# bennevans/mjrl

Hardware: AMD Instinct MI355X
Metric: NPG train_step timesteps/sec, Humanoid 1M-step batch @ 1/2/4/8 MI355X (higher is better)
Workload: dtype f32 (split-f16 MFMA, f32 accumulate); 1 GPU; humanoid_npg_1M; obs_dim=376, act_dim=17, algo=npg, horizon=1000, cg_iters=10, parallelism=dp1, comm=LocalComm

## Files before the change

### mjrl_amd/csrc/common.h

```cpp
#pragma once

#include <hip/hip_runtime.h>
#include <stdint.h>

#include "../../include/mjrl_amd.h"

#ifdef MJRL_KX_PROF
constexpr int KX_NPROF = 24;
__device__ unsigned long long g_kx_prof[KX_NPROF];
#define KX_STAMP(i)                                                     \
    do {                                                                \
        const unsigned long long now_ = __builtin_amdgcn_s_memtime();   \
        kx_acc_[i] += now_ - kx_last_;                                  \
        kx_last_ = now_;                                                \
    } while (0)
#define KX_PRE(i) kx_pre_[i] = __builtin_amdgcn_s_memtime()
#else
#define KX_PRE(i) \
    do {          \
    } while (0)
#define KX_STAMP(i) \
    do {            \
    } while (0)
#endif

namespace mjrl {

typedef float floatx4 __attribute__((ext_vector_type(4)));

constexpr int WAVE = 64;
constexpr int NTHREADS = 256;

__device__ __forceinline__ floatx4 zero4() { return floatx4{0.f, 0.f, 0.f, 0.f}; }

__device__ __forceinline__ floatx4 mfma4(float a, float b, floatx4 c) {
    return __builtin_amdgcn_mfma_f32_16x16x4f32(a, b, c, 0, 0, 0);
}

__device__ __forceinline__ floatx4 mfma_k16(const float4& a, const float4& b, floatx4 c) {
    c = mfma4(a.x, b.x, c);
    c = mfma4(a.y, b.y, c);
    c = mfma4(a.z, b.z, c);
    c = mfma4(a.w, b.w, c);
    return c;
}

typedef _Float16 half8 __attribute__((ext_vector_type(8)));
typedef short short4v __attribute__((ext_vector_type(4)));

__device__ __forceinline__ floatx4 mfma_h(const half8& a, const half8& b, floatx4 c) {
    return __builtin_amdgcn_mfma_f32_16x16x32_f16(a, b, c, 0, 0, 0);
}

__device__ __forceinline__ floatx4 mfma_x3(const half8& ah, const half8& al, const half8& bh, const half8& bl,
                                           floatx4 c) {
    c = mfma_h(ah, bh, c);
    c = mfma_h(ah, bl, c);
    return mfma_h(al, bh, c);
}

constexpr int SPLIT_HR = 15;

__device__ __forceinline__ float pow2_scale(float M, float& inv) {
    if (!(M > 0.f) || !(M < 3.0e38f)) {
        inv = 1.f;
        return 1.f;
    }
    int E;
    frexpf(M, &E);
    E = E < -111 ? -111 : E;
    inv = ldexpf(1.f, E - SPLIT_HR);
    return ldexpf(1.f, SPLIT_HR - E);
}

__device__ __forceinline__ float col_scale(float cmax) {
    if (!(cmax > 0.f) || !(cmax < 3.0e38f)) return 1.f;
    int E;
    frexpf(cmax, &E);
    E = E < -100 ? -100 : (E > 100 ? 100 : E);
    return ldexpf(1.f, E);
}

constexpr float AHR = 16384.f;
constexpr float AHR_INV = 1.f / 16384.f;

typedef float float8v __attribute__((ext_vector_type(8)));
typedef short short8v __attribute__((ext_vector_type(8)));

typedef unsigned uint4v __attribute__((ext_vector_type(4)));

__device__ __forceinline__ uint4v mix_lo8(const uint4v& h, const float8v& y) {
    uint4v l;
    asm("v_fma_mixlo_f16 %0, %4, -1.0, %8 op_sel_hi:[1,0,0]\n\t"
        "v_fma_mixhi_f16 %0, %4, -1.0, %9 op_sel:[1,0,0] op_sel_hi:[1,0,0]\n\t"
        "v_fma_mixlo_f16 %1, %5, -1.0, %10 op_sel_hi:[1,0,0]\n\t"
        "v_fma_mixhi_f16 %1, %5, -1.0, %11 op_sel:[1,0,0] op_sel_hi:[1,0,0]\n\t"
        "v_fma_mixlo_f16 %2, %6, -1.0, %12 op_sel_hi:[1,0,0]\n\t"
        "v_fma_mixhi_f16 %2, %6, -1.0, %13 op_sel:[1,0,0] op_sel_hi:[1,0,0]\n\t"
        "v_fma_mixlo_f16 %3, %7, -1.0, %14 op_sel_hi:[1,0,0]\n\t"
        "v_fma_mixhi_f16 %3, %7, -1.0, %15 op_sel:[1,0,0] op_sel_hi:[1,0,0]\n\t"
        "s_nop 1"
        : "=&v"(l[0]), "=&v"(l[1]), "=&v"(l[2]), "=&v"(l[3])
        : "v"(h[0]), "v"(h[1]), "v"(h[2]), "v"(h[3]), "v"(y[0]), "v"(y[1]), "v"(y[2]), "v"(y[3]), "v"(y[4]),
          "v"(y[5]), "v"(y[6]), "v"(y[7]));
    return l;
}

__device__ __forceinline__ unsigned mix_lo2(unsigned hi2, float y0, float y1) {
    unsigned t;
    asm("v_fma_mixlo_f16 %0, %1, -1.0, %2 op_sel_hi:[1,0,0]\n\t"
        "v_fma_mixhi_f16 %0, %1, -1.0, %3 op_sel:[1,0,0] op_sel_hi:[1,0,0]"
        : "=&v"(t) : "v"(hi2), "v"(y0), "v"(y1));
    return t;
}

__device__ __forceinline__ void split8(const float8v& v, float s, half8& hi, half8& lo) {
    const float8v y = v * s;
    hi = __builtin_convertvector(y, half8);
    lo = __builtin_bit_cast(half8, mix_lo8(__builtin_bit_cast(uint4v, hi), y));
}

__device__ __forceinline__ float mix_add_lo(unsigned h2, unsigned l2) {
    float r;
    asm("v_fma_mix_f32 %0, %1, 1.0, %2 op_sel_hi:[1,0,1]" : "=v"(r) : "v"(h2), "v"(l2));
    return r;
}
__device__ __forceinline__ float mix_add_hi(unsigned h2, unsigned l2) {
    float r;
    asm("v_fma_mix_f32 %0, %1, 1.0, %2 op_sel:[1,0,1] op_sel_hi:[1,0,1]" : "=v"(r) : "v"(h2), "v"(l2));
    return r;
}
__device__ __forceinline__ float8v hilo8(const half8& hh, const half8& ll) {
    const uint4v h = __builtin_bit_cast(uint4v, hh), l = __builtin_bit_cast(uint4v, ll);
    float8v r;
#pragma unroll
    for (int p = 0; p < 4; ++p) {
        r[2 * p] = mix_add_lo(h[p], l[p]);
        r[2 * p + 1] = mix_add_hi(h[p], l[p]);
    }
    return r;
}

__device__ __forceinline__ float8v load8(const float* p) {
    const float4 a = *reinterpret_cast<const float4*>(p);
    const float4 b = *reinterpret_cast<const float4*>(p + 4);
    return float8v{a.x, a.y, a.z, a.w, b.x, b.y, b.z, b.w};
}

__device__ __forceinline__ float absmax8(const float8v& v) {
    float m = 0.f;
#pragma unroll
    for (int e = 0; e < 8; ++e) m = fmaxf(m, fabsf(v[e]));
    return m;
}

__device__ __forceinline__ float max_over_groups(float v) {
    const auto a = __builtin_amdgcn_permlane16_swap(__float_as_uint(v), __float_as_uint(v), false, false);
    v = fmaxf(__uint_as_float(a[0]), __uint_as_float(a[1]));
    const auto b = __builtin_amdgcn_permlane32_swap(__float_as_uint(v), __float_as_uint(v), false, false);
    return fmaxf(__uint_as_float(b[0]), __uint_as_float(b[1]));
}

__device__ __forceinline__ float sum_over_groups(float v) {
    const auto a = __builtin_amdgcn_permlane16_swap(__float_as_uint(v), __float_as_uint(v), false, false);
    v = __uint_as_float(a[0]) + __uint_as_float(a[1]);
    const auto b = __builtin_amdgcn_permlane32_swap(__float_as_uint(v), __float_as_uint(v), false, false);
    return __uint_as_float(b[0]) + __uint_as_float(b[1]);
}

__device__ __forceinline__ short4v ds_read_tr16(const void* p) {
    typedef __attribute__((address_space(3))) short4v lds_short4;
    return __builtin_amdgcn_ds_read_tr16_b64_v4i16((lds_short4*)(p));
}

template <int RB, int CB, int NW = 4>
struct Split {
    static constexpr int WPC = CB >= NW ? 1 : NW / CB;
    static constexpr int NCW = CB >= NW ? CB / NW : 1;
    static constexpr int NRW = CB >= NW ? RB : (RB + WPC - 1) / WPC;
    static constexpr int CBS = CB >= NW ? NW : 1;
    static constexpr int RBS = CB >= NW ? 1 : WPC;
    __device__ static int cb0(int w) { return CB >= NW ? w : w % CB; }
    __device__ static int rb0(int w) { return CB >= NW ? 0 : w / CB; }
};

template <int NRW, int NCW>
__device__ __forceinline__ void gemm_tile(floatx4 (&acc)[NRW][NCW], const float* As, int lda, int a_col0,
                                          int rb0, int rbs, int rb_lim, const float* __restrict__ W, int ldw,
                                          int cb0, int cbs, int kb, int ke, int lane) {
    const int r = lane & 15, q = lane >> 4;
#ifndef MJRL_GEMM_UNROLL
#define MJRL_GEMM_UNROLL 8
#endif
#pragma unroll MJRL_GEMM_UNROLL
    for (int k = kb; k < ke; k += 16) {
        float4 b[NCW];
#pragma unroll
        for (int j = 0; j < NCW; ++j)
            b[j] = *reinterpret_cast<const float4*>(W + (size_t)((cb0 + j * cbs) * 16 + r) * ldw + k + 4 * q);
#pragma unroll
        for (int i = 0; i < NRW; ++i) {
            const int rb = rb0 + i * rbs;
            if (rb >= rb_lim) continue;
            const float4 a = *reinterpret_cast<const float4*>(As + (rb * 16 + r) * lda + (k - a_col0) + 4 * q);
#pragma unroll
            for (int j = 0; j < NCW; ++j) acc[i][j] = mfma_k16(a, b[j], acc[i][j]);
        }
    }
}

template <int NRW, int NCW>
__device__ __forceinline__ void zero_acc(floatx4 (&acc)[NRW][NCW]) {
#pragma unroll
// ... 174 lines not shown
```

### mjrl_amd/csrc/kx.h

```cpp
#pragma once


namespace {

constexpr int AIMG_BYTES = 64 * 64;

template <int MP, int KG>
struct XLayout {
    static constexpr int H = 64, BT = 32;
    static constexpr int NP = 32 * KG, KH = NP / 2;
    static constexpr int RBYTES = NP * 2;
    static constexpr int LD = H + 4;
    static constexpr int LDT = BT + 4;
    static constexpr int LDG = 32 + 4;
    static constexpr int WIMG = 64 * 128;
    static constexpr int WIMG2 = 32 * 128;
    static constexpr int AIMG = AIMG_BYTES;
    static constexpr int oXH = 0;
    static constexpr int oXL = oXH + BT * RBYTES;
    static constexpr int oS1 = oXL + BT * RBYTES;
    static constexpr int oS2 = oS1 + 2 * WIMG;
    static constexpr int oS3 = oS2 + 2 * WIMG;
    static constexpr int oS4 = oS3 + 2 * WIMG2;
    static constexpr int oSC = oS4 + 2 * WIMG2;
    static constexpr int oU = oSC + (64 + 64 + 64 + 32) * 4;
    static constexpr int oD0 = oU + BT * 4;
    static constexpr int oD1 = oD0 + BT * LD * 4;
    static constexpr int D1SZ = (BT * LD > H * LDT ? BT * LD : H * LDT) * 4;
    static constexpr int oGP = oD1 + D1SZ;
    static constexpr int oGPT = oGP + BT * LDG * 4;
    static constexpr int oG1T = oGPT + 32 * LDT * 4;
    static constexpr int oA0 = oG1T + H * LDT * 4;
    static constexpr int oA1 = oA0 + 2 * AIMG;
    static constexpr int oD0B = oA1 + 2 * AIMG;
    static constexpr int bytes = oD0B + BT * LD * 4;
    static_assert(bytes <= 160 * 1024, "LDS");
    static_assert(bytes >= 2 * KT * 8, "row_pass_final scratch");
    static constexpr int XPER = BT * NP / 4 / KT;
    static_assert(NP % 128 == 0, "chunk swizzle of the xhat images");
    static_assert(MP == 16 || MP == 32, "output layer: one k32 step");
};

__device__ __forceinline__ int swz128(int r) { return (((r >> 1) & 1) << 1) | (((r >> 3) & 1) << 2); }
__device__ __forceinline__ int woff(int row, int col) { return row * 128 + 16 * ((col >> 3) ^ swz128(row)) + 2 * (col & 7); }
__device__ __forceinline__ int aoff(int f, int row) { return f * 64 + 16 * ((row >> 3) ^ (((f >> 3) & 1) << 1)) + 2 * (row & 7); }

template <int CTRL>
__device__ __forceinline__ float dpp_f(float x) {
    return __int_as_float(__builtin_amdgcn_update_dpp(__float_as_int(x), __float_as_int(x), CTRL, 0xf, 0xf, false));
}
__device__ __forceinline__ float row16_max(float v) {
    v = fmaxf(v, dpp_f<0xB1>(v));
    v = fmaxf(v, dpp_f<0x4E>(v));
    v = fmaxf(v, dpp_f<0x141>(v));
    return fmaxf(v, dpp_f<0x140>(v));
}

__device__ __forceinline__ half8 cat_tr(const short4v& a, const short4v& b) {
    return __builtin_bit_cast(half8, __builtin_shufflevector(a, b, 0, 1, 2, 3, 4, 5, 6, 7));
}

__device__ __forceinline__ void wrow(const char* img, int imgbytes, int j, int s, int q, half8& h, half8& l) {
    const int off = woff(j, 32 * s + 8 * q);
    h = *reinterpret_cast<const half8*>(img + off);
    l = *reinterpret_cast<const half8*>(img + imgbytes + off);
}
__device__ __forceinline__ void wcol(const char* img, int imgbytes, int hb, int s, int q, int r, half8& h, half8& l) {
    const int tq = r >> 2, tp = r & 3;
    const int o0 = woff(32 * s + 8 * q + tq, hb * 16 + 4 * tp);
    const int o1 = woff(32 * s + 8 * q + 4 + tq, hb * 16 + 4 * tp);
    h = cat_tr(ds_read_tr16(img + o0), ds_read_tr16(img + o1));
    l = cat_tr(ds_read_tr16(img + imgbytes + o0), ds_read_tr16(img + imgbytes + o1));
}
__device__ __forceinline__ void arow(const char* img, int rb, int s, int q, int r, half8& h, half8& l) {
    const int tq = r >> 2, tp = r & 3;
    const int o0 = aoff(32 * s + 8 * q + tq, rb * 16 + 4 * tp);
    const int o1 = aoff(32 * s + 8 * q + 4 + tq, rb * 16 + 4 * tp);
    h = cat_tr(ds_read_tr16(img + o0), ds_read_tr16(img + o1));
    l = cat_tr(ds_read_tr16(img + AIMG_BYTES + o0), ds_read_tr16(img + AIMG_BYTES + o1));
}
__device__ __forceinline__ void acol(const char* img, int f, int q, half8& h, half8& l) {
    const int off = aoff(f, 8 * q);
    h = *reinterpret_cast<const half8*>(img + off);
    l = *reinterpret_cast<const half8*>(img + AIMG_BYTES + off);
}
__device__ __forceinline__ void aval4(const char* img, int f, int row0, float (&v)[4]) {
    typedef unsigned uint2v __attribute__((ext_vector_type(2)));
    const int off = aoff(f, row0);
    const uint2v h = *reinterpret_cast<const uint2v*>(img + off);
    const uint2v l = *reinterpret_cast<const uint2v*>(img + AIMG_BYTES + off);
    v[0] = mix_add_lo(h[0], l[0]) * AHR_INV;
    v[1] = mix_add_hi(h[0], l[0]) * AHR_INV;
    v[2] = mix_add_lo(h[1], l[1]) * AHR_INV;
    v[3] = mix_add_hi(h[1], l[1]) * AHR_INV;
}
__device__ __forceinline__ void astore4(char* img, int f, int row0, const float (&a)[4]) {
    typedef _Float16 half4 __attribute__((ext_vector_type(4)));
    typedef unsigned uint2v __attribute__((ext_vector_type(2)));
    typedef float float4v __attribute__((ext_vector_type(4)));
    const float v[4] = {a[0] * AHR, a[1] * AHR, a[2] * AHR, a[3] * AHR};
    const float4v x = {v[0], v[1], v[2], v[3]};
    const half4 h = __builtin_convertvector(x, half4);
    const uint2v hb = __builtin_bit_cast(uint2v, h);
    const uint2v lb = {mix_lo2(hb[0], v[0], v[1]), mix_lo2(hb[1], v[2], v[3])};
    const int off = aoff(f, row0);
    *reinterpret_cast<uint2v*>(img + off) = hb;
    *reinterpret_cast<uint2v*>(img + AIMG_BYTES + off) = lb;
}

template <int KS>
__device__ __forceinline__ float adyn(const float* buf, int ld, int rb, int q, int r, const float* fold,
                                      half8 (&h)[KS], half8 (&l)[KS]) {
    float8v v[KS];
    float mx = 0.f;
#pragma unroll
    for (int s = 0; s < KS; ++s) {
        v[s] = load8(buf + (rb * 16 + r) * ld + 32 * s + 8 * q);
        if (fold) v[s] *= load8(fold + 32 * s + 8 * q);
        mx = fmaxf(mx, absmax8(v[s]));
    }
    float inv;
    const float sc = pow2_scale(max_over_groups(mx), inv);
#pragma unroll
    for (int s = 0; s < KS; ++s) split8(v[s], sc, h[s], l[s]);
    return inv;
}

__device__ __forceinline__ void gdyn(const float* bufT, int ldt, int ub, int q, int r, half8& h, half8& l,
                                     float (&sc4)[4]) {
    const float8v v = load8(bufT + (ub * 16 + r) * ldt + 8 * q);
    float inv;
    const float s = pow2_scale(max_over_groups(absmax8(v)), inv);
    split8(v, s, h, l);
#pragma unroll
    for (int rr = 0; rr < 4; ++rr) sc4[rr] = __shfl(inv, 4 * q + rr, 64);
}

template <int IR>
__device__ __forceinline__ void wload(const float* __restrict__ W, int nrows, float (&v)[IR], int tid) {
    const int lane = tid & 63, w = tid >> 6;
#pragma unroll
    for (int k = 0; k < IR; ++k) {
        const int j = w + 8 * k;
        v[k] = j < nrows ? W[j * 64 + lane] : 0.f;
    }
}

template <bool COLS, int IR>
__device__ __forceinline__ void wscale(const float (&v)[IR], float* inv, float* red, int tid) {
    const int lane = tid & 63, w = tid >> 6;
    if (COLS) {
        float mx = 0.f;
#pragma unroll
        for (int k = 0; k < IR; ++k) mx = fmaxf(mx, fabsf(v[k]));
        red[w * 64 + lane] = mx;
    } else {
#pragma unroll
        for (int k = 0; k < IR; ++k) {
            float mx = fabsf(v[k]);
#pragma unroll
            for (int o = 32; o > 0; o >>= 1) mx = fmaxf(mx, __shfl_xor(mx, o, 64));
            float iv;
            pow2_scale(mx, iv);
            if (lane == 0) inv[w + 8 * k] = iv;
        }
    }
}

__device__ __forceinline__ void wscale_cols(float* inv, const float* red, int tid) {
    if (tid < 64) {
        float mx = 0.f;
#pragma unroll
        for (int i = 0; i < KT / 64; ++i) mx = fmaxf(mx, red[i * 64 + tid]);
        float iv;
        pow2_scale(mx, iv);
        inv[tid] = iv;
    }
}

template <int NR>
__device__ __forceinline__ float8v wload_rows(const float* __restrict__ W, int nrows, int tid) {
    const int j = tid >> 3;
    float8v v = {0.f, 0.f, 0.f, 0.f, 0.f, 0.f, 0.f, 0.f};
    if (j < NR && j < nrows) v = load8(W + j * 64 + 8 * (tid & 7));
    return v;
}
template <int NR>
__device__ __forceinline__ void wrows_store(const float8v& v, char* img, int imgbytes, float* inv, int tid) {
    float mx = absmax8(v);
    mx = fmaxf(mx, __shfl_xor(mx, 1, 64));
    mx = fmaxf(mx, __shfl_xor(mx, 2, 64));
    mx = fmaxf(mx, __shfl_xor(mx, 4, 64));
    const int j = tid >> 3;
    if (j < NR) {
        float iv;
        const float sc = pow2_scale(mx, iv);
        half8 h, l;
        split8(v, sc, h, l);
        const int off = j * 128 + 16 * ((tid & 7) ^ swz128(j));
        *reinterpret_cast<half8*>(img + off) = h;
        *reinterpret_cast<half8*>(img + imgbytes + off) = l;
        if ((tid & 7) == 0) inv[j] = iv;
    }
}

template <bool COLS, int IR>
__device__ __forceinline__ void wstore(const float (&v)[IR], char* img, int imgbytes, const float* inv, int tid) {
    const int lane = tid & 63, w = tid >> 6;
#pragma unroll
    for (int k = 0; k < IR; ++k) {
        const int j = w + 8 * k;
        const float y = v[k] * __builtin_amdgcn_rcpf(inv[COLS ? lane : j]);
        const _Float16 h = (_Float16)y;
        const int off = woff(j, lane);
        *reinterpret_cast<_Float16*>(img + off) = h;
        *reinterpret_cast<_Float16*>(img + imgbytes + off) = (_Float16)(y - (float)h);
    }
}

#ifdef MJRL_KX_ABL_NOCHAIN
constexpr bool KX_ABL_NOCHAIN = true;
#else
constexpr bool KX_ABL_NOCHAIN = false;
#endif
#ifdef MJRL_KX_ABL_NOCOLS
constexpr bool KX_ABL_NOCOLS = true;
#else
constexpr bool KX_ABL_NOCOLS = false;
#endif

template <int MP, int KG, int MODE, bool PACK = false>
__global__ void __launch_bounds__(KT, 1) k_kx(RowArgs a, FOut o) {
#pragma clang fp contract(fast)
    using L = XLayout<MP, KG>;
    constexpr int H = 64, BT = L::BT, NP = L::NP, KH = L::KH;
    constexpr bool GRAD = MODE != EVAL;
    extern __shared__ __attribute__((aligned(16))) float smem[];
    char* sb = reinterpret_cast<char*>(smem);
    char* XHb = sb + L::oXH;
    char* XLb = sb + L::oXL;
    char* S1 = sb + L::oS1;
    char* S2 = sb + L::oS2;
    char* S3 = sb + L::oS3;
    char* S4 = sb + L::oS4;
    float* sc1 = reinterpret_cast<float*>(sb + L::oSC);
    float* sc2 = sc1 + 64;
    float* sc3 = sc2 + 64;
    float* sc4v = sc3 + 64;
    float* Us = reinterpret_cast<float*>(sb + L::oU);
    float* D0 = reinterpret_cast<float*>(sb + L::oD0);
    float* D0B = reinterpret_cast<float*>(sb + L::oD0B);
    float* D1 = reinterpret_cast<float*>(sb + L::oD1);
    float* GPf = reinterpret_cast<float*>(sb + L::oGP);
    float* GPT = reinterpret_cast<float*>(sb + L::oGPT);
    float* G1T = reinterpret_cast<float*>(sb + L::oG1T);
    char* A0i = sb + L::oA0;
    char* A1i = sb + L::oA1;

#ifdef MJRL_KX_PROF
    const unsigned long long kx_t0_ = __builtin_amdgcn_s_memtime();
    unsigned long long kx_pre_[6];
#endif
    const int tid = threadIdx.x, lane = tid & 63, w = __builtin_amdgcn_readfirstlane(tid >> 6);
    const int r16 = lane & 15, q = lane >> 4;
    const int cb = w & 3, kh = w >> 2;
    const int m = a.m;
    const int64_t T = a.T;
    const int64_t ntiles = (T + BT - 1) / BT;
    const float* P = a.P;
    const Packed pk(H, H, NP, MP);
    const float* W0src = (MODE == FVP ? a.V : P) + pk.W0;


    constexpr int KS = KH / 32;
    static_assert(KT == 512 && MP <= 32, "preamble layout: 8 waves, output-layer images of 32 rows");
    float w1v[8], w3v[4];
    float8v rv1, rv2;
    if (MODE == EVAL) {
        rv1 = wload_rows<64>(P + pk.W1, H, tid);
        rv2 = wload_rows<32>(P + pk.W2, MP, tid);
    } else {
        wload(P + pk.W1, H, w1v, tid);
        wload(P + pk.W2, MP, w3v, tid);
        const float* src = MODE == FVP ? a.V : P;
        rv1 = wload_rows<64>(src + pk.W1, H, tid);
        rv2 = wload_rows<32>(src + pk.W2, MP, tid);
    }
    const float* BV = MODE == FVP ? a.V : P;
    const float bias1 = BV[pk.b1 + cb * 16 + r16];
    const int cbo3 = w & (MP / 16 - 1), rb3 = w / (MP / 16);
    const int col3 = cbo3 * 16 + r16;
    const float bias3 = BV[pk.b2 + col3];
    const float os3 = a.out_scale ? (col3 < m ? a.out_scale[col3] : 1.f) : 1.f;
    const float osh3 = a.out_shift ? (col3 < m ? a.out_shift[col3] : 0.f) : 0.f;
    float wq3 = 0.f;
    if (MODE == FVP) {
        const float sg = expf(P[pk.ls + col3]);
        wq3 = os3 * os3 * (2.f / (2.f * sg * sg + 1e-8f));
    }
    const float sls = MODE == FVP ? 0.f : ls_sum(P + pk.ls, m);
    RowConst rconst{};
    if constexpr (MODE != FVP) rconst = row_const<MODE, MP>(a, P + pk.ls, tid);
    KX_PRE(0);
    half8 wh[KS], wl[KS];
    float wsc;
    {
        float8v v[KS];
#pragma unroll
        for (int s = 0; s < KS; ++s) {
            const int k0 = kh * KH + 32 * s + 8 * q;
            v[s] = load8(W0src + (cb * 16 + r16) * NP + k0) * load8(a.xc + k0);
        }
        float mx = 0.f;
#pragma unroll
        for (int s = 0; s < KS; ++s) mx = fmaxf(mx, absmax8(v[s]));
        const float sc = pow2_scale(max_over_groups(mx), wsc);
#pragma unroll
        for (int s = 0; s < KS; ++s) split8(v[s], sc, wh[s], wl[s]);
// ... 12 lines not shown
                wscale<true>(w1v, sc1, red1, tid);
                wscale<true>(w3v, sc3, red3, tid);
            }
        }
        KX_PRE(2);
        if (MODE != EVAL && !(KX_ABL_NOCOLS && MODE == FVP)) {
            __syncthreads();
            wscale_cols(sc1, red1, tid);
            wscale_cols(sc3, red3, tid);
            __syncthreads();
        }
        KX_PRE(3);
        if (MODE != EVAL) {
            wstore<true>(w1v, S1, L::WIMG, sc1, tid);
            wstore<true>(w3v, S3, L::WIMG2, sc3, tid);
        }
    }
    KX_PRE(4);
    float* picx = D0B;
    if constexpr (PACK) {
        static_assert(MODE == FWD, "the fused pack is the forward pass's");
        static_assert(NP * 4 <= L::BT * L::LD * 4, "pack table in the D0B region");
        for (int k = tid; k < NP; k += KT) picx[k] = 1.f / a.xc[k];
    }
    if ((MODE == FVP || MODE == EVAL) && a.done && *a.done) return;

    floatx4 g0[KG];
#pragma unroll
    for (int g = 0; g < KG; ++g) g0[g] = zero4();
    floatx4 g1[2] = {zero4(), zero4()};
    floatx4 g2 = zero4();
    float b1acc = 0.f, b2acc = 0.f;
    double racc0 = 0.0, racc1 = 0.0;


    float touch[2] = {0.f, 0.f};
    float4 xn[L::XPER];
    float un = 1.f;
    auto xload = [&](int64_t t_, int tid_, int u0 = 0, int u1 = L::XPER) {
        const int64_t rb_ = t_ * BT;
        const int row = tid_ >> 4, c16 = tid_ & 15;
        const bool ok = t_ < ntiles && rb_ + row < T;
        if constexpr (PACK) {
            const float* src = a.obs32 + (ok ? (rb_ + row) * (int64_t)a.n_obs : 0);
#pragma unroll
            for (int u = 0; u < L::XPER; ++u)
                if (u >= u0 && u < u1) {
                    const int col = 8 * (c16 + 16 * (u >> 1)) + 4 * (u & 1);
                    xn[u] = ok && col < a.n_obs ? *reinterpret_cast<const float4*>(src + col)
                                                : make_float4(0.f, 0.f, 0.f, 0.f);
                }
            return;
        }
        const char* src = reinterpret_cast<const char*>(a.xs) + (ok ? (rb_ + row) * (4 * NP) : 0);
#pragma unroll
        for (int u = 0; u < L::XPER; ++u)
            if (u >= u0 && u < u1)
                xn[u] = ok ? *reinterpret_cast<const float4*>(src + 16 * (c16 + 16 * u)) : make_float4(0.f, 0.f, 0.f, 0.f);
        if (u0 == 0) {
            const bool uok = tid_ < BT && t_ < ntiles && rb_ + tid_ < T;
            un = a.xu[uok ? rb_ + tid_ : 0];
        }
    };
    xload(blockIdx.x, tid);
    __syncthreads();
#ifdef MJRL_KX_PROF
    unsigned long long kx_acc_[KX_NPROF] = {0};
    unsigned long long kx_last_ = __builtin_amdgcn_s_memtime();
    kx_acc_[15] = kx_last_ - kx_t0_;
    kx_acc_[17] = 1;
    kx_acc_[18] = kx_pre_[0] - kx_t0_;
    for (int i = 1; i < 5; ++i) kx_acc_[18 + i] = kx_pre_[i] - kx_pre_[i - 1];
    kx_acc_[23] = kx_last_ - kx_pre_[4];
#endif

    const float wsc1 = MODE == FVP ? wsc * sc1[cb * 16 + r16] : wsc;
#ifndef MJRL_KX_OFFREG
    const int p1A = 16 * (kh * (KH / 8) + q), p1B = 16 * chunk_swz(r16), p1C = r16 * L::RBYTES;
    auto p1off_at = [&](int s, int opq_) { return (((p1A + opq_) + 64 * s) ^ p1B) + p1C; };
#else
    int p1off[KS];
#pragma unroll
    for (int s = 0; s < KS; ++s) p1off[s] = r16 * L::RBYTES + 16 * ((kh * (KH / 8) + 4 * s + q) ^ chunk_swz(r16));
    auto p1off_at = [&](int s, int) { return p1off[s]; };
#endif
    auto gw0_off = [&](int r_, int q_, int g) {
        const int tq = r_ >> 2, tp = r_ & 3, row = 8 * q_ + tq;
        return row * L::RBYTES + 16 * (((kh * KH) / 8 + (tp >> 1) + 2 * g) ^ chunk_swz(row)) + 8 * (tp & 1);
    };
#ifndef MJRL_KX_OFFREG
    const int g0row = 8 * q + (r16 >> 2);
    const int g0A = 16 * ((kh * KH) / 8 + ((r16 & 3) >> 1)), g0B = 16 * chunk_swz(g0row),
              g0C = g0row * L::RBYTES + 8 * (r16 & 1);
    auto g0off_at = [&](int g, int opq_) { return (((g0A + opq_) + 32 * g) ^ g0B) + g0C; };
#else
    int g0off[MODE != EVAL ? KG : 1];
    if constexpr (MODE != EVAL) {
#pragma unroll
        for (int g = 0; g < KG; ++g) g0off[g] = gw0_off(r16, q, g);
    }
    auto g0off_at = [&](int g, int) { return g0off[g]; };
#endif
    for (int64_t tile = blockIdx.x; tile < ntiles; tile += gridDim.x) {
        KX_STAMP(9);
        int opq = 0;
        if constexpr (MODE != EVAL) asm volatile("" : "+v"(opq));
        constexpr int OPQ_LANE = MODE == FWD ? 1 : 0;
// ... 9 lines not shown
            const bool ok = row < nrow;
            float8v v[UH];
            float mx = 0.f;
#pragma unroll
            for (int c = 0; c < UH; ++c) {
                const int c0 = 8 * (c16 + 16 * c);
                v[c] = float8v{xn[2 * c].x, xn[2 * c].y, xn[2 * c].z, xn[2 * c].w,
                               xn[2 * c + 1].x, xn[2 * c + 1].y, xn[2 * c + 1].z, xn[2 * c + 1].w};
                const float8v ic = load8(picx + c0);
#pragma unroll
                for (int e = 0; e < 8; ++e) {
                    if (c0 + e == a.n_obs && ok) v[c][e] = 1.f;
                    v[c][e] *= ic[e];
                }
                mx = fmaxf(mx, absmax8(v[c]));
            }
            mx = row16_max(mx);
            float inv;
            const float sc = pow2_scale(mx, inv);
            char* dst = XHb + row * L::RBYTES + 16 * (c16 ^ chunk_swz(row));
            _Float16* gdst = a.xs_w + (row_base + row) * (2 * (int64_t)NP);
#pragma unroll
            for (int c = 0; c < UH; ++c) {
                half8 h, l;
                split8(v[c], sc, h, l);
                *reinterpret_cast<half8*>(dst + 256 * c) = h;
                *reinterpret_cast<half8*>(dst + BT * L::RBYTES + 256 * c) = l;
                if (ok) {
                    const int c0 = 8 * (c16 + 16 * c);
                    *reinterpret_cast<half8*>(gdst + c0) = h;
                    *reinterpret_cast<half8*>(gdst + NP + c0) = l;
                }
            }
            if (c16 == 0) {
                Us[row] = inv;
                if (ok) a.xu_w[row_base + row] = inv;
            }
        } else {
            const int row = ltid >> 4, c16 = ltid & 15;
            char* dst = XHb + row * L::RBYTES + 16 * (c16 ^ chunk_swz(row));
#pragma unroll
            for (int u = 0; u < L::XPER; ++u) {
                constexpr int UH = NP / 128;
                *reinterpret_cast<float4*>(dst + (u / UH) * (BT * L::RBYTES) + 256 * (u % UH)) = xn[u];
            }
            if (ltid < BT) Us[ltid] = un;
        }
        if (MODE == EVAL) xload(tile + gridDim.x, ltid);
        float pa0[4], pa1[4];
        if (MODE == FVP) {
#pragma unroll
            for (int rr = 0; rr < 4; ++rr) {
                const int row = kh * 16 + 4 * lq + rr;
                const int64_t gi = (row_base + (row < nrow ? row : 0)) * H + cb * 16 + lr16;
                pa0[rr] = a.a0[gi];
                pa1[rr] = a.a1[gi];
            }
        }
        __syncthreads();
        KX_STAMP(0);
        RowPre<BT, MP, KT> rpre;
        if constexpr (MODE == EVAL) row_pre_load<MODE, BT, MP, KT>(a, row_base, ltid, rpre);
        {
            const int64_t nt = tile + gridDim.x;
            if (nt < ntiles) {
                const int64_t nb = nt * BT;
                const int nr = (int)(T - nb < BT ? T - nb : BT);
                const int mline = (BT * m * 4 + 127) / 128;
                const int idx = ltid;
                const float* p = nullptr;
                if (MODE == FVP) {
                    if (idx < 4 * BT && (idx & 63) / 2 < nr)
                        p = (idx < 2 * BT ? a.a0 : a.a1) + (nb + (idx & 63) / 2) * H + (idx & 1) * 32;
                } else {
                    const int ne = nr * m;
                    if (idx < mline) {
                        if (32 * idx < ne) p = a.act + nb * m + 32 * idx;
                    } else if (MODE == EVAL && idx < 2 * mline) {
                        if (32 * (idx - mline) < ne) p = a.mu0 + nb * m + 32 * (idx - mline);
                    } else if (idx == 2 * mline) {
                        p = (MODE == FWD ? a.adv_vpg : a.adv) + nb;
                    } else if (MODE == EVAL && idx == 2 * mline + 1) {
                        p = a.ll0 + nb;
                    }
                }
                touch[0] = *(p ? p : reinterpret_cast<const float*>(a.xs));
            } else {
                touch[0] = *reinterpret_cast<const float*>(a.xs);
            }
        }

        floatx4 acc1[2] = {zero4(), zero4()};
#ifdef MJRL_KX_ABL_NOP1
        if (MODE != FVP)
#endif
        {
#pragma unroll
            for (int s = 0; s < KS; ++s) {
#pragma unroll
                for (int i = 0; i < 2; ++i) {
                    const int off = p1off_at(s, opq) + i * 16 * L::RBYTES;
                    const half8 xh = *reinterpret_cast<const half8*>(XHb + off);
                    const half8 xl = *reinterpret_cast<const half8*>(XLb + off);
                    acc1[i] = mfma_x3(xh, xl, wh[s], wl[s], acc1[i]);
                }
                if (s % 3 == 2) __builtin_amdgcn_sched_barrier(0);
            }
#pragma unroll
            for (int i = 0; i < 2; ++i)
#pragma unroll
                for (int rr = 0; rr < 4; ++rr) acc1[i][rr] *= Us[i * 16 + 4 * lq + rr] * wsc1;
        }
        if (MODE == FVP) {
            float* dst = kh ? D0B : D0;
#pragma unroll
            for (int i = 0; i < 2; ++i)
#pragma unroll
                for (int rr = 0; rr < 4; ++rr) dst[(i * 16 + 4 * lq + rr) * L::LD + cb * 16 + lr16] = acc1[i][rr];
            astore4(A0i, cb * 16 + lr16, kh * 16 + 4 * lq, pa0);
            astore4(A1i, cb * 16 + lr16, kh * 16 + 4 * lq, pa1);
            __syncthreads();
            KX_STAMP(1);
            KX_STAMP(2);
        } else {
#pragma unroll
            for (int rr = 0; rr < 4; ++rr)
                D0[((1 - kh) * 16 + 4 * lq + rr) * L::LD + cb * 16 + lr16] = kh ? acc1[0][rr] : acc1[1][rr];
            __syncthreads();
            KX_STAMP(1);
            {
                const int col = cb * 16 + lr16;
                float av[4];
#pragma unroll
                for (int rr = 0; rr < 4; ++rr) {
                    const int row = kh * 16 + 4 * lq + rr;
                    av[rr] = tanhf((kh ? acc1[1][rr] : acc1[0][rr]) + D0[row * L::LD + col]);
                    if (MODE == FWD && row < nrow) a.a0[(row_base + row) * H + col] = av[rr];
                }
                astore4(A0i, col, kh * 16 + 4 * lq, av);
            }
            __syncthreads();
            KX_STAMP(2);
        }

        if (!(KX_ABL_NOCHAIN && MODE == FVP)) {
            const int j = cb * 16 + lr16;
            floatx4 acc = zero4();
            float rinv = 1.f;
            if (MODE == FVP) {
                half8 xh[2], xl[2], ah[2], al[2];
                float8v dv[2];
                float mx = 0.f;
#pragma unroll
                for (int s = 0; s < 2; ++s) {
                    arow(A0i, kh, s, lq, lr16, xh[s], xl[s]);
                    const int o = (kh * 16 + lr16) * L::LD + 32 * s + 8 * lq;
                    const float8v av = hilo8(xh[s], xl[s]) * AHR_INV;
                    dv[s] = (load8(D0 + o) + load8(D0B + o)) * (1.f - av * av);
                    mx = fmaxf(mx, absmax8(dv[s]));
                }
                const float sc = pow2_scale(max_over_groups(mx), rinv);
                float ri[4];
#pragma unroll
                for (int rr = 0; rr < 4; ++rr) ri[rr] = __shfl(rinv, 4 * lq + rr, 64);
                floatx4 accb = zero4();
#pragma unroll
                for (int s = 0; s < 2; ++s) {
                    split8(dv[s], sc, ah[s], al[s]);
                    half8 bh, bl;
                    wrow(S1, L::WIMG, j, s, lq, bh, bl);
                    acc = mfma_x3(ah[s], al[s], bh, bl, acc);
                    wrow(S2, L::WIMG, j, s, lq, bh, bl);
                    accb = mfma_x3(xh[s], xl[s], bh, bl, accb);
                }
                const float dsc = sc2[j] * AHR_INV;
#pragma unroll
                for (int rr = 0; rr < 4; ++rr) acc[rr] = acc[rr] * ri[rr] + accb[rr] * dsc;
            } else {
                const char* img = MODE == FWD ? S2 : S1;
#pragma unroll
                for (int s = 0; s < 2; ++s) {
                    half8 bh, bl, xh, xl;
                    arow(A0i, kh, s, lq, lr16, xh, xl);
                    wrow(img, L::WIMG, j, s, lq, bh, bl);
                    acc = mfma_x3(xh, xl, bh, bl, acc);
                }
                const float rsc = (MODE == FWD ? sc2 : sc1)[j] * AHR_INV;
#pragma unroll
                for (int rr = 0; rr < 4; ++rr) acc[rr] *= rsc;
            }
            float av[4];
#pragma unroll
            for (int rr = 0; rr < 4; ++rr) {
                const int row = kh * 16 + 4 * lq + rr;
                const float v = acc[rr] + bias1;
                if (MODE == FVP) {
                    D1[row * L::LD + j] = (1.f - pa1[rr] * pa1[rr]) * v;
                } else {
                    av[rr] = tanhf(v);
                    if (MODE == FWD && row < nrow) a.a1[(row_base + row) * H + j] = av[rr];
                }
            }
            if (MODE != FVP) astore4(A1i, j, kh * 16 + 4 * lq, av);
        }
        __syncthreads();
        KX_STAMP(3);

        if (w < 2 * (MP / 16) && !(KX_ABL_NOCHAIN && MODE == FVP)) {
            floatx4 acc = zero4();
            if (MODE == FVP) {
                half8 ah[2], al[2];
                const float rinv = adyn<2>(D1, L::LD, rb3, lq, lr16, sc3, ah, al);
                float ri[4];
#pragma unroll
                for (int rr = 0; rr < 4; ++rr) ri[rr] = __shfl(rinv, 4 * lq + rr, 64);
                floatx4 accb = zero4();
#pragma unroll
                for (int s = 0; s < 2; ++s) {
                    half8 bh, bl, xh, xl;
                    wrow(S3, L::WIMG2, col3, s, lq, bh, bl);
                    acc = mfma_x3(ah[s], al[s], bh, bl, acc);
                    arow(A1i, rb3, s, lq, lr16, xh, xl);
                    wrow(S4, L::WIMG2, col3, s, lq, bh, bl);
                    accb = mfma_x3(xh, xl, bh, bl, accb);
                }
                const float dsc = sc4v[col3] * AHR_INV;
#pragma unroll
                for (int rr = 0; rr < 4; ++rr) acc[rr] = acc[rr] * ri[rr] + accb[rr] * dsc;
            } else {
                const char* img = MODE == FWD ? S4 : S3;
#pragma unroll
                for (int s = 0; s < 2; ++s) {
                    half8 bh, bl, xh, xl;
                    arow(A1i, rb3, s, lq, lr16, xh, xl);
                    wrow(img, L::WIMG2, col3, s, lq, bh, bl);
                    acc = mfma_x3(xh, xl, bh, bl, acc);
                }
                const float rsc = (MODE == FWD ? sc4v : sc3)[col3] * AHR_INV;
#pragma unroll
                for (int rr = 0; rr < 4; ++rr) acc[rr] *= rsc;
            }
            float gv[4];
#pragma unroll
            for (int rr = 0; rr < 4; ++rr) {
                const int row = rb3 * 16 + 4 * lq + rr;
                const float v = acc[rr] + bias3;
                if (MODE == FVP)
                    gv[rr] = (col3 < m && row < nrow) ? wq3 * v : 0.f;
                else
                    gv[rr] = col3 < m ? v * os3 + osh3 : 0.f;
                GPf[row * L::LDG + col3] = gv[rr];
            }
            if (MODE == FVP)
                *reinterpret_cast<float4*>(GPT + col3 * L::LDT + rb3 * 16 + 4 * lq) =
                    make_float4(gv[0], gv[1], gv[2], gv[3]);
        }
        if (MP == 16) {
            for (int i = ltid; i < BT * 16; i += KT) GPf[(i >> 4) * L::LDG + 16 + (i & 15)] = 0.f;
        }
        __syncthreads();
        KX_STAMP(4);

        if (MODE == EVAL) {
            row_pass<MODE, BT, MP, KT, false, true>(a, P + pk.ls, sls, row_base, GPf, L::LDG, racc0, racc1, ltid,
                                                    &rpre, &rconst);
            __syncthreads();
            KX_STAMP(5);
            continue;
        }
        if (MODE != FVP) {
            row_pass<MODE, BT, MP, KT, false>(a, P + pk.ls, sls, row_base, GPf, L::LDG, racc0, racc1, ltid,
                                              nullptr, &rconst);
            __syncthreads();
        KX_STAMP(5);
            if (MODE == EVAL) continue;
            for (int i = ltid; i < BT * MP; i += KT) {
                const int row = i / MP, jj = i % MP;
                GPT[jj * L::LDT + row] = GPf[row * L::LDG + jj];
            }
        }
        if (MODE == EVAL) continue;

        xload(tile + gridDim.x, ltid, 0, L::XPER / 2);
        if (!(KX_ABL_NOCHAIN && MODE == FVP)) {
            const int hcol = cb * 16 + lr16;
            half8 ah[1], al[1];
            const float rinv = adyn<1>(GPf, L::LDG, kh, lq, lr16, nullptr, ah, al);
            float ri[4];
#pragma unroll
            for (int rr = 0; rr < 4; ++rr) ri[rr] = __shfl(rinv, 4 * lq + rr, 64);
            half8 bh, bl;
            wcol(S3, L::WIMG2, cb, 0, lq, lr16, bh, bl);
            const floatx4 acc = mfma_x3(ah[0], al[0], bh, bl, zero4());
            const float csc = sc3[hcol];
            float gv[4], a4[4];
            if (MODE != FVP) aval4(A1i, hcol, kh * 16 + 4 * lq, a4);
#pragma unroll
            for (int rr = 0; rr < 4; ++rr) {
                const int row = kh * 16 + 4 * lq + rr;
                const float av = MODE == FVP ? pa1[rr] : a4[rr];
                gv[rr] = (1.f - av * av) * (acc[rr] * ri[rr] * csc);
                D0[row * L::LD + hcol] = gv[rr];
            }
            *reinterpret_cast<float4*>(G1T + hcol * L::LDT + kh * 16 + 4 * lq) = make_float4(gv[0], gv[1], gv[2], gv[3]);
        }
        auto gw2_sum = [&]() __attribute__((always_inline)) {
            half8 gh, gl;
            float s4[4];
            if ((w >> 2) < MP / 16) {
                const float8v v = load8(GPT + ((w >> 2) * 16 + lr16) * L::LDT + 8 * lq);
                float inv;
                const float sc = pow2_scale(max_over_groups(absmax8(v)), inv);
                split8(v, sc, gh, gl);
#pragma unroll
                for (int rr = 0; rr < 4; ++rr) s4[rr] = __shfl(inv * AHR_INV, 4 * lq + rr, 64);
                if ((w & 3) == 0) {
                    b2acc += sum_over_groups(((v[0] + v[1]) + (v[2] + v[3])) + ((v[4] + v[5]) + (v[6] + v[7])));
                }
                half8 bh, bl;
                acol(A1i, (w & 3) * 16 + lr16, lq, bh, bl);
                const floatx4 t = mfma_x3(gh, gl, bh, bl, zero4());
#pragma unroll
                for (int rr = 0; rr < 4; ++rr) g2[rr] += t[rr] * s4[rr];
            }
        };
        if (MODE == FVP && !KX_ABL_NOCHAIN) gw2_sum();
        __syncthreads();
        KX_STAMP(6);
        xload(tile + gridDim.x, ltid, L::XPER / 2, L::XPER);
        auto p5_gu0 = [&]() __attribute__((always_inline)) {
            const int hcol = cb * 16 + lr16;
            half8 ah[2], al[2];
            const float rinv = adyn<2>(D0, L::LD, kh, lq, lr16, nullptr, ah, al);
            float ri[4];
#pragma unroll
            for (int rr = 0; rr < 4; ++rr) ri[rr] = __shfl(rinv, 4 * lq + rr, 64);
            floatx4 acc = zero4();
#pragma unroll
            for (int s = 0; s < 2; ++s) {
                half8 bh, bl;
                wcol(S1, L::WIMG, cb, s, lq, lr16, bh, bl);
                acc = mfma_x3(ah[s], al[s], bh, bl, acc);
            }
            const float csc = sc1[hcol];
            float gv[4], a4[4];
            aval4(A0i, hcol, kh * 16 + 4 * lq, a4);
#pragma unroll
            for (int rr = 0; rr < 4; ++rr) {
                const int row = kh * 16 + 4 * lq + rr;
                const float av = a4[rr];
                gv[rr] = (1.f - av * av) * (acc[rr] * ri[rr] * csc) * Us[row];
            }
            *reinterpret_cast<float4*>(D1 + hcol * L::LDT + kh * 16 + 4 * lq) = make_float4(gv[0], gv[1], gv[2], gv[3]);
        };
        auto p5_gw = [&]() __attribute__((always_inline)) {
            half8 gh, gl;
            float s4[4];
            {
                const float8v v = load8(G1T + (cb * 16 + lr16) * L::LDT + 8 * lq);
                float inv;
                const float sc = pow2_scale(max_over_groups(absmax8(v)), inv);
                split8(v, sc, gh, gl);
#pragma unroll
                for (int rr = 0; rr < 4; ++rr) s4[rr] = __shfl(inv * AHR_INV, 4 * lq + rr, 64);
                if (kh == 0) {
                    b1acc += sum_over_groups(((v[0] + v[1]) + (v[2] + v[3])) + ((v[4] + v[5]) + (v[6] + v[7])));
                }
            }
#pragma unroll
            for (int jj = 0; jj < 2; ++jj) {
                half8 bh, bl;
                acol(A0i, (kh + 2 * jj) * 16 + lr16, lq, bh, bl);
                const floatx4 t = mfma_x3(gh, gl, bh, bl, zero4());
#pragma unroll
                for (int rr = 0; rr < 4; ++rr) g1[jj][rr] += t[rr] * s4[rr];
            }
        };
        if (!(KX_ABL_NOCHAIN && MODE == FVP)) {
            p5_gu0();
            p5_gw();
        }
        if (MODE != FVP) gw2_sum();
        __syncthreads();
        KX_STAMP(7);

        KX_STAMP(10);
#ifdef MJRL_KX_ABL_NOP6
        if (false)
#endif
        {
            half8 gh, gl;
            float s4[4];
            gdyn(D1, L::LDT, cb, lq, lr16, gh, gl, s4);
            KX_STAMP(11);
#pragma unroll
            for (int g = 0; g < KG; ++g) {
                short4v th[2], tl[2];
#pragma unroll
                for (int h = 0; h < 2; ++h) {
                    const int off = g0off_at(g, opq) + h * 4 * L::RBYTES;
                    th[h] = ds_read_tr16(XHb + off);
                    tl[h] = ds_read_tr16(XLb + off);
                }
                const floatx4 t = mfma_x3(gh, gl, cat_tr(th[0], th[1]), cat_tr(tl[0], tl[1]), zero4());
#pragma unroll
                for (int rr = 0; rr < 4; ++rr) g0[g][rr] += t[rr] * s4[rr];
                if (g & 1) __builtin_amdgcn_sched_barrier(0);
            }
            KX_STAMP(12);
        }
        KX_STAMP(14);
        __syncthreads();
        KX_STAMP(8);
    }

    const int64_t blk = blockIdx.x;
    if constexpr (GRAD) {
        const int n = o.n, mm = o.m;
        const int64_t S = gridDim.x;
        float* slab = smem;
        static_assert(H * NP + H + H * H + H + MP * H + MP <= L::bytes / 4, "slab staging in LDS");
        auto put = [&](int f, float v) { slab[f] = v; };
        const int fb0 = H * n, fW1 = fb0 + H, fb1 = fW1 + H * H, fW2 = fb1 + H, fb2 = fW2 + mm * H;
#pragma unroll
        for (int g = 0; g < KG; ++g) {
            const int k = kh * KH + 16 * g + r16;
            const float xck = a.xc[k];
#pragma unroll
            for (int rr = 0; rr < 4; ++rr) {
                const int hid = cb * 16 + 4 * q + rr;
                if (k < n)
                    put(hid * n + k, g0[g][rr] * xck);
                else if (k == n)
                    put(fb0 + hid, g0[g][rr] * xck);
            }
        }
#pragma unroll
        for (int j = 0; j < 2; ++j)
#pragma unroll
            for (int rr = 0; rr < 4; ++rr) put(fW1 + (cb * 16 + 4 * q + rr) * H + (kh + 2 * j) * 16 + r16, g1[j][rr]);
        if ((w >> 2) < MP / 16) {
#pragma unroll
            for (int rr = 0; rr < 4; ++rr) {
                const int j = (w >> 2) * 16 + 4 * q + rr;
                if (j < mm) put(fW2 + j * H + (w & 3) * 16 + r16, g2[rr]);
            }
// ... 32 lines not shown
```

Measured before the change: 95.80 million timesteps/s.

## Cache 1-a^2 factors, replace shuffles with LDS broadcast, bit-trick pow2 scale

Computes the tanh-derivative factors (1-a^2) once when storing activations, keeping them in registers or in an LDS scratch region instead of recomputing them from split-f16 images. Replaces per-lane __shfl broadcasts of scale factors with a per-wave LDS scratch write and float4 read. Rewrites pow2_scale with integer exponent bit manipulation, switches max reductions to unsigned-bit compares, and narrows some global index arithmetic to 32-bit offsets. The aim is to cut VALU and cross-lane work in the FVP kernel, at the cost of extra LDS traffic and a little more LDS footprint. The pow2_scale namespace change may need call-site qualification.

```diff
diff --git a/mjrl_amd/csrc/common.h b/mjrl_amd/csrc/common.h
--- a/mjrl_amd/csrc/common.h
+++ b/mjrl_amd/csrc/common.h
@@ -4,6 +4,7 @@
 #include <stdint.h>
 
 #include "../../include/mjrl_amd.h"
+#include "pow2_scale.h"
 
 #ifdef MJRL_KX_PROF
 constexpr int KX_NPROF = 24;
@@ -59,19 +60,6 @@
     return mfma_h(al, bh, c);
 }
 
-constexpr int SPLIT_HR = 15;
-
-__device__ __forceinline__ float pow2_scale(float M, float& inv) {
-    if (!(M > 0.f) || !(M < 3.0e38f)) {
-        inv = 1.f;
-        return 1.f;
-    }
-    int E;
-    frexpf(M, &E);
-    E = E < -111 ? -111 : E;
-    inv = ldexpf(1.f, E - SPLIT_HR);
-    return ldexpf(1.f, SPLIT_HR - E);
-}
 
 __device__ __forceinline__ float col_scale(float cmax) {
     if (!(cmax > 0.f) || !(cmax < 3.0e38f)) return 1.f;
@@ -130,17 +118,6 @@
     asm("v_fma_mix_f32 %0, %1, 1.0, %2 op_sel:[1,0,1] op_sel_hi:[1,0,1]" : "=v"(r) : "v"(h2), "v"(l2));
     return r;
 }
-__device__ __forceinline__ float8v hilo8(const half8& hh, const half8& ll) {
-    const uint4v h = __builtin_bit_cast(uint4v, hh), l = __builtin_bit_cast(uint4v, ll);
-    float8v r;
-#pragma unroll
-    for (int p = 0; p < 4; ++p) {
-        r[2 * p] = mix_add_lo(h[p], l[p]);
-        r[2 * p + 1] = mix_add_hi(h[p], l[p]);
-    }
-    return r;
-}
-
 __device__ __forceinline__ float8v load8(const float* p) {
     const float4 a = *reinterpret_cast<const float4*>(p);
     const float4 b = *reinterpret_cast<const float4*>(p + 4);
@@ -154,11 +131,15 @@
     return m;
 }
 
+__device__ __forceinline__ float umax_bits(float a, float b) {
+    const unsigned x = __float_as_uint(a), y = __float_as_uint(b);
+    return __uint_as_float(x > y ? x : y);
+}
 __device__ __forceinline__ float max_over_groups(float v) {
     const auto a = __builtin_amdgcn_permlane16_swap(__float_as_uint(v), __float_as_uint(v), false, false);
-    v = fmaxf(__uint_as_float(a[0]), __uint_as_float(a[1]));
-    const auto b = __builtin_amdgcn_permlane32_swap(__float_as_uint(v), __float_as_uint(v), false, false);
-    return fmaxf(__uint_as_float(b[0]), __uint_as_float(b[1]));
+    const unsigned m = a[0] > a[1] ? a[0] : a[1];
+    const auto b = __builtin_amdgcn_permlane32_swap(m, m, false, false);
+    return __uint_as_float(b[0] > b[1] ? b[0] : b[1]);
 }
 
 __device__ __forceinline__ float sum_over_groups(float v) {
diff --git a/mjrl_amd/csrc/kx.h b/mjrl_amd/csrc/kx.h
--- a/mjrl_amd/csrc/kx.h
+++ b/mjrl_amd/csrc/kx.h
@@ -33,7 +33,8 @@
     static constexpr int oA0 = oG1T + H * LDT * 4;
     static constexpr int oA1 = oA0 + 2 * AIMG;
     static constexpr int oD0B = oA1 + 2 * AIMG;
-    static constexpr int bytes = oD0B + BT * LD * 4;
+    static constexpr int oBC = oD0B + BT * LD * 4;
+    static constexpr int bytes = oBC + (KT / 64) * 16 * 4;
     static_assert(bytes <= 160 * 1024, "LDS");
     static_assert(bytes >= 2 * KT * 8, "row_pass_final scratch");
     static constexpr int XPER = BT * NP / 4 / KT;
@@ -50,10 +51,10 @@
     return __int_as_float(__builtin_amdgcn_update_dpp(__float_as_int(x), __float_as_int(x), CTRL, 0xf, 0xf, false));
 }
 __device__ __forceinline__ float row16_max(float v) {
-    v = fmaxf(v, dpp_f<0xB1>(v));
-    v = fmaxf(v, dpp_f<0x4E>(v));
-    v = fmaxf(v, dpp_f<0x141>(v));
-    return fmaxf(v, dpp_f<0x140>(v));
+    v = umax_bits(v, dpp_f<0xB1>(v));
+    v = umax_bits(v, dpp_f<0x4E>(v));
+    v = umax_bits(v, dpp_f<0x141>(v));
+    return umax_bits(v, dpp_f<0x140>(v));
 }
 
 __device__ __forceinline__ half8 cat_tr(const short4v& a, const short4v& b) {
@@ -107,6 +108,35 @@
     *reinterpret_cast<uint2v*>(img + off) = hb;
     *reinterpret_cast<uint2v*>(img + AIMG_BYTES + off) = lb;
 }
+__device__ __forceinline__ void astore4_om(char* img, int f, int row0, const float (&a)[4], float (&om)[4]) {
+    typedef _Float16 half4 __attribute__((ext_vector_type(4)));
+    typedef unsigned uint2v __attribute__((ext_vector_type(2)));
+    typedef float float4v __attribute__((ext_vector_type(4)));
+    const float v[4] = {a[0] * AHR, a[1] * AHR, a[2] * AHR, a[3] * AHR};
+    const float4v x = {v[0], v[1], v[2], v[3]};
+    const half4 h = __builtin_convertvector(x, half4);
+    const uint2v hb = __builtin_bit_cast(uint2v, h);
+    const uint2v lb = {mix_lo2(hb[0], v[0], v[1]), mix_lo2(hb[1], v[2], v[3])};
+    const int off = aoff(f, row0);
+    *reinterpret_cast<uint2v*>(img + off) = hb;
+    *reinterpret_cast<uint2v*>(img + AIMG_BYTES + off) = lb;
+    const float av[4] = {mix_add_lo(hb[0], lb[0]) * AHR_INV, mix_add_hi(hb[0], lb[0]) * AHR_INV,
+                         mix_add_lo(hb[1], lb[1]) * AHR_INV, mix_add_hi(hb[1], lb[1]) * AHR_INV};
+#pragma unroll
+    for (int rr = 0; rr < 4; ++rr) om[rr] = __builtin_fmaf(-av[rr], av[rr], 1.f);
+}
+
+__device__ __forceinline__ void bcast4(float* scr, float inv, int q, int r, float (&o)[4]) {
+    scr[r] = inv;
+    __builtin_amdgcn_fence(__ATOMIC_RELEASE, "wavefront");
+    __builtin_amdgcn_wave_barrier();
+    __builtin_amdgcn_fence(__ATOMIC_ACQUIRE, "wavefront");
+    const float4 t = *reinterpret_cast<const float4*>(scr + 4 * q);
+    o[0] = t.x;
+    o[1] = t.y;
+    o[2] = t.z;
+    o[3] = t.w;
+}
 
 template <int KS>
 __device__ __forceinline__ float adyn(const float* buf, int ld, int rb, int q, int r, const float* fold,
@@ -127,13 +157,12 @@
 }
 
 __device__ __forceinline__ void gdyn(const float* bufT, int ldt, int ub, int q, int r, half8& h, half8& l,
-                                     float (&sc4)[4]) {
+                                     float (&sc4)[4], float* scr) {
     const float8v v = load8(bufT + (ub * 16 + r) * ldt + 8 * q);
     float inv;
     const float s = pow2_scale(max_over_groups(absmax8(v)), inv);
     split8(v, s, h, l);
-#pragma unroll
-    for (int rr = 0; rr < 4; ++rr) sc4[rr] = __shfl(inv, 4 * q + rr, 64);
+    bcast4(scr, inv, q, r, sc4);
 }
 
 template <int IR>
@@ -218,6 +247,10 @@
     }
 }
 
+#ifndef MJRL_KX_OM_REG
+#define MJRL_KX_OM_REG 1
+#endif
+constexpr bool KX_OM_REG = MJRL_KX_OM_REG;
 #ifdef MJRL_KX_ABL_NOCHAIN
 constexpr bool KX_ABL_NOCHAIN = true;
 #else
@@ -254,6 +287,8 @@
     float* GPf = reinterpret_cast<float*>(sb + L::oGP);
     float* GPT = reinterpret_cast<float*>(sb + L::oGPT);
     float* G1T = reinterpret_cast<float*>(sb + L::oG1T);
+    float* OM = G1T;
+    static_assert(BT * L::LD <= H * L::LDT, "OM in the G1T region");
     char* A0i = sb + L::oA0;
     char* A1i = sb + L::oA1;
 
@@ -264,6 +299,7 @@
     const int tid = threadIdx.x, lane = tid & 63, w = __builtin_amdgcn_readfirstlane(tid >> 6);
     const int r16 = lane & 15, q = lane >> 4;
     const int cb = w & 3, kh = w >> 2;
+    float* bcs = reinterpret_cast<float*>(sb + L::oBC) + w * 16;
     const int m = a.m;
     const int64_t T = a.T;
     const int64_t ntiles = (T + BT - 1) / BT;
@@ -382,7 +418,7 @@
                 }
             return;
         }
-        const char* src = reinterpret_cast<const char*>(a.xs) + (ok ? (rb_ + row) * (4 * NP) : 0);
+        const char* src = reinterpret_cast<const char*>(a.xs) + rb_ * (4 * NP) + (ok ? (unsigned)(row * (4 * NP)) : 0u);
 #pragma unroll
         for (int u = 0; u < L::XPER; ++u)
             if (u >= u0 && u < u1)
@@ -498,9 +534,9 @@
 #pragma unroll
             for (int rr = 0; rr < 4; ++rr) {
                 const int row = kh * 16 + 4 * lq + rr;
-                const int64_t gi = (row_base + (row < nrow ? row : 0)) * H + cb * 16 + lr16;
-                pa0[rr] = a.a0[gi];
-                pa1[rr] = a.a1[gi];
+                const unsigned gi = (unsigned)((row < nrow ? row : 0) * H + cb * 16 + lr16);
+                pa0[rr] = (a.a0 + row_base * H)[gi];
+                pa1[rr] = (a.a1 + row_base * H)[gi];
             }
         }
         __syncthreads();
@@ -563,8 +599,12 @@
             for (int i = 0; i < 2; ++i)
 #pragma unroll
                 for (int rr = 0; rr < 4; ++rr) dst[(i * 16 + 4 * lq + rr) * L::LD + cb * 16 + lr16] = acc1[i][rr];
-            astore4(A0i, cb * 16 + lr16, kh * 16 + 4 * lq, pa0);
+            astore4_om(A0i, cb * 16 + lr16, kh * 16 + 4 * lq, pa0, pa0);
+#pragma unroll
+            for (int rr = 0; rr < 4; ++rr) OM[(kh * 16 + 4 * lq + rr) * L::LD + cb * 16 + lr16] = pa0[rr];
             astore4(A1i, cb * 16 + lr16, kh * 16 + 4 * lq, pa1);
+#pragma unroll
+            for (int rr = 0; rr < 4; ++rr) pa1[rr] = __builtin_fmaf(-pa1[rr], pa1[rr], 1.f);
             __syncthreads();
             KX_STAMP(1);
             KX_STAMP(2);
@@ -601,14 +641,12 @@
                 for (int s = 0; s < 2; ++s) {
                     arow(A0i, kh, s, lq, lr16, xh[s], xl[s]);
                     const int o = (kh * 16 + lr16) * L::LD + 32 * s + 8 * lq;
-                    const float8v av = hilo8(xh[s], xl[s]) * AHR_INV;
-                    dv[s] = (load8(D0 + o) + load8(D0B + o)) * (1.f - av * av);
+                    dv[s] = (load8(D0 + o) + load8(D0B + o)) * load8(OM + o);
                     mx = fmaxf(mx, absmax8(dv[s]));
                 }
                 const float sc = pow2_scale(max_over_groups(mx), rinv);
                 float ri[4];
-#pragma unroll
-                for (int rr = 0; rr < 4; ++rr) ri[rr] = __shfl(rinv, 4 * lq + rr, 64);
+                bcast4(bcs, rinv, lq, lr16, ri);
                 floatx4 accb = zero4();
 #pragma unroll
                 for (int s = 0; s < 2; ++s) {
@@ -641,7 +679,7 @@
                 const int row = kh * 16 + 4 * lq + rr;
                 const float v = acc[rr] + bias1;
                 if (MODE == FVP) {
-                    D1[row * L::LD + j] = (1.f - pa1[rr] * pa1[rr]) * v;
+                    D1[row * L::LD + j] = pa1[rr] * v;
                 } else {
                     av[rr] = tanhf(v);
                     if (MODE == FWD && row < nrow) a.a1[(row_base + row) * H + j] = av[rr];
@@ -658,8 +696,7 @@
                 half8 ah[2], al[2];
                 const float rinv = adyn<2>(D1, L::LD, rb3, lq, lr16, sc3, ah, al);
                 float ri[4];
-#pragma unroll
-                for (int rr = 0; rr < 4; ++rr) ri[rr] = __shfl(rinv, 4 * lq + rr, 64);
+                bcast4(bcs, rinv, lq, lr16, ri);
                 floatx4 accb = zero4();
 #pragma unroll
                 for (int s = 0; s < 2; ++s) {
@@ -733,8 +770,7 @@
             half8 ah[1], al[1];
             const float rinv = adyn<1>(GPf, L::LDG, kh, lq, lr16, nullptr, ah, al);
             float ri[4];
-#pragma unroll
-            for (int rr = 0; rr < 4; ++rr) ri[rr] = __shfl(rinv, 4 * lq + rr, 64);
+            bcast4(bcs, rinv, lq, lr16, ri);
             half8 bh, bl;
             wcol(S3, L::WIMG2, cb, 0, lq, lr16, bh, bl);
             const floatx4 acc = mfma_x3(ah[0], al[0], bh, bl, zero4());
@@ -744,8 +780,8 @@
 #pragma unroll
             for (int rr = 0; rr < 4; ++rr) {
                 const int row = kh * 16 + 4 * lq + rr;
-                const float av = MODE == FVP ? pa1[rr] : a4[rr];
-                gv[rr] = (1.f - av * av) * (acc[rr] * ri[rr] * csc);
+                const float om = MODE == FVP ? pa1[rr] : 1.f - a4[rr] * a4[rr];
+                gv[rr] = om * (acc[rr] * ri[rr] * csc);
                 D0[row * L::LD + hcol] = gv[rr];
             }
             *reinterpret_cast<float4*>(G1T + hcol * L::LDT + kh * 16 + 4 * lq) = make_float4(gv[0], gv[1], gv[2], gv[3]);
@@ -758,8 +794,7 @@
                 float inv;
                 const float sc = pow2_scale(max_over_groups(absmax8(v)), inv);
                 split8(v, sc, gh, gl);
-#pragma unroll
-                for (int rr = 0; rr < 4; ++rr) s4[rr] = __shfl(inv * AHR_INV, 4 * lq + rr, 64);
+                bcast4(bcs, inv * AHR_INV, lq, lr16, s4);
                 if ((w & 3) == 0) {
                     b2acc += sum_over_groups(((v[0] + v[1]) + (v[2] + v[3])) + ((v[4] + v[5]) + (v[6] + v[7])));
                 }
@@ -779,8 +814,7 @@
             half8 ah[2], al[2];
             const float rinv = adyn<2>(D0, L::LD, kh, lq, lr16, nullptr, ah, al);
             float ri[4];
-#pragma unroll
-            for (int rr = 0; rr < 4; ++rr) ri[rr] = __shfl(rinv, 4 * lq + rr, 64);
+            bcast4(bcs, rinv, lq, lr16, ri);
             floatx4 acc = zero4();
 #pragma unroll
             for (int s = 0; s < 2; ++s) {
@@ -790,12 +824,13 @@
             }
             const float csc = sc1[hcol];
             float gv[4], a4[4];
-            aval4(A0i, hcol, kh * 16 + 4 * lq, a4);
+            constexpr bool OMREG = MODE == FVP && KX_OM_REG && !(MP == 16 && KG == 12);
+            if (!OMREG) aval4(A0i, hcol, kh * 16 + 4 * lq, a4);
 #pragma unroll
             for (int rr = 0; rr < 4; ++rr) {
                 const int row = kh * 16 + 4 * lq + rr;
-                const float av = a4[rr];
-                gv[rr] = (1.f - av * av) * (acc[rr] * ri[rr] * csc) * Us[row];
+                const float om = OMREG ? pa0[rr] : 1.f - a4[rr] * a4[rr];
+                gv[rr] = om * (acc[rr] * ri[rr] * csc) * Us[row];
             }
             *reinterpret_cast<float4*>(D1 + hcol * L::LDT + kh * 16 + 4 * lq) = make_float4(gv[0], gv[1], gv[2], gv[3]);
         };
@@ -807,8 +842,7 @@
                 float inv;
                 const float sc = pow2_scale(max_over_groups(absmax8(v)), inv);
                 split8(v, sc, gh, gl);
-#pragma unroll
-                for (int rr = 0; rr < 4; ++rr) s4[rr] = __shfl(inv * AHR_INV, 4 * lq + rr, 64);
+                bcast4(bcs, inv * AHR_INV, lq, lr16, s4);
                 if (kh == 0) {
                     b1acc += sum_over_groups(((v[0] + v[1]) + (v[2] + v[3])) + ((v[4] + v[5]) + (v[6] + v[7])));
                 }
@@ -837,7 +871,7 @@
         {
             half8 gh, gl;
             float s4[4];
-            gdyn(D1, L::LDT, cb, lq, lr16, gh, gl, s4);
+            gdyn(D1, L::LDT, cb, lq, lr16, gh, gl, s4, bcs);
             KX_STAMP(11);
 #pragma unroll
             for (int g = 0; g < KG; ++g) {
diff --git a/mjrl_amd/csrc/pow2_scale.h b/mjrl_amd/csrc/pow2_scale.h
--- /dev/null
+++ b/mjrl_amd/csrc/pow2_scale.h
@@ -0,0 +1,37 @@
+#pragma once
+
+#include <stdint.h>
+
+#ifdef __HIPCC__
+#define MJRL_HD __host__ __device__ inline __attribute__((always_inline))
+#else
+#define MJRL_HD inline
+#endif
+
+namespace mjrl {
+
+constexpr int SPLIT_HR = 15;
+
+MJRL_HD uint32_t f32_bits(float x) {
+    uint32_t u;
+    __builtin_memcpy(&u, &x, 4);
+    return u;
+}
+MJRL_HD float bits_f32(uint32_t u) {
+    float x;
+    __builtin_memcpy(&x, &u, 4);
+    return x;
+}
+
+MJRL_HD float pow2_scale(float M, float& inv) {
+    constexpr uint32_t EXP = 0x7F800000u, LIM = 0x7F61B1E6u;
+    constexpr uint32_t EMIN = 15u << 23, ONE = 141u << 23;
+    const uint32_t u = f32_bits(M);
+    uint32_t t = u & EXP;
+    t = t < EMIN ? EMIN : t;
+    t = u - 1u < LIM - 1u ? t : ONE;
+    inv = bits_f32(t - (14u << 23));
+    return bits_f32((268u << 23) - t);
+}
+
+}
```

Result: faster. 98.10 million timesteps/s (median of 6 runs) (+2.4%).
